# mhvk/baseband-tasks

Measured on AMD Instinct MI355X. Metric: Msamples/s through Dedisperse(DM=100)+Channelize(1k ch), 2-pol c64, higher is better.
Workload: dtype c64; 1 GPU; configs[1]+metric pipeline: Dedisperse DM=100, 16 MHz BW at 1000 MHz, 2^20-sample overlap-save blocks (836100 valid) -> Channelize(1024), 2-pol complex64, HBM-resident input; n_fft=1048576, n_chan=1024, streams_per_gpu=2, outputs=left sharded on the ranks (value); with_gather includes the all-gather

## Files before the change

### baseband-tasks_amd/csrc/bbt_hip.hip

```cpp
#include <hip/hip_runtime.h>
#include <dlfcn.h>
#include <rccl/rccl.h>

#include <algorithm>
#include <chrono>
#include <cmath>
#include <cstdarg>
#include <cstdio>
#include <cstdlib>
#include <cstring>
#include <initializer_list>
#include <map>
#include <mutex>
#include <string>
#include <tuple>
#include <vector>

#include "../../include/bbt_hip.h"
#include "bbt_kernels.hpp"
#include "gen_kernels.hpp"
#include "big_kernels.hpp"
#include "gen2_host.hpp"
#include "gen_host.hpp"
#include "osm_geo.hpp"
// ... 644 lines not shown
    int n2p = 0;
    long long in_plane = 0, out_plane = 0;
    float2* seam = nullptr;
    float2* seam_buf[2] = {nullptr, nullptr};
    size_t seam_bytes[2] = {0, 0};
    OsmKnobs knobs;
    std::vector<OsmLaunch> chunk_launches;

    bool timing = false;
    bool timing_isolated = false;
    std::vector<hipEvent_t> ev;
    std::vector<hipEvent_t> ev_free;
    int timing_stride = 4;
    int64_t pass_launches[3] = {0, 0, 0};
    int64_t pass_blocks[3] = {0, 0, 0};
    std::vector<int> ev_nblk;
    double acc_ms[3] = {0, 0, 0};
    int64_t launches = 0;
};

static int osm_flush_timing(bbt_osm_plan* p) {
    for (size_t i = 0; i + 3 < p->ev.size(); i += 4) {
        HIP_TRY(hipEventSynchronize(p->ev[i + 3]));
        for (int k = 0; k < 3; ++k) {
            float ms = 0.f;
            HIP_TRY(hipEventElapsedTime(&ms, p->ev[i + k], p->ev[i + k + 1]));
            p->acc_ms[k] += ms;
            p->pass_launches[k] += 1;
            p->pass_blocks[k] += p->ev_nblk[i / 4];
        }
        p->launches += 1;
    }
    for (auto e : p->ev) p->ev_free.push_back(e);
    p->ev.clear();
    p->ev_nblk.clear();
    return 0;
}

static_assert(fft_lds_elems(256) == FftGeo<256>::LDS_ELEMS && fft_lds_elems(512) == FftGeo<512>::LDS_ELEMS &&
                  fft_lds_elems(1024) == FftGeo<1024>::LDS_ELEMS && fft_lds_elems(2048) == FftGeo<2048>::LDS_ELEMS &&
                  fft_lds_elems(4096) == FftGeo<4096>::LDS_ELEMS && big_lds_elems(8192) == BigGeo<8192>::LDS_ELEMS &&
                  big_lds_elems(16384) == BigGeo<16384>::LDS_ELEMS && sizeof(v2) == 8 && sizeof(f4) == 16,
              "osm_launch.hpp: the exchange areas are not the templates'");

static int osm_dispatch(bbt_osm_plan* p, const OsmLaunch& l, const float2* in, float2* out, float2* work,
                        const OsmChunk& ch, const OsmChunk& chw, const SpecOut& so, hipStream_t st) {
    const dim3 grid(l.gx, l.gy), block(l.threads);
    const int S = l.single ? 1 : p->S;
#define BBT_GO(KERNEL_, ...)                                                      \
    {                                                                             \
        if (l.raise_lds && ensure_dyn_lds((const void*)KERNEL_, l.lds)) return 1; \
        hipLaunchKernelGGL(KERNEL_, grid, block, l.lds, st, __VA_ARGS__);         \
        return 0;                                                                 \
    }
    switch (l.family) {
        case OSM_COL16:
#define BBT_COL16(FIRST_, SPEC_, SINGLE_, PP_)                                      \
    if (l.first == FIRST_ && l.spec == SPEC_ && l.single == SINGLE_ && l.pp == PP_) \
        BBT_GO((k_osm_col16<FIRST_, SPEC_, SINGLE_, PP_>), in, out, work, ch, S, p->n2, so)
            BBT_COL16(true, false, true, 1) BBT_COL16(true, false, false, 8) BBT_COL16(true, false, false, 1)
            BBT_COL16(false, true, true, 1) BBT_COL16(false, false, true, 1) BBT_COL16(false, true, false, 8)
            BBT_COL16(false, false, false, 8) BBT_COL16(false, true, false, 1) BBT_COL16(false, false, false, 1)
#undef BBT_COL16
            break;
        case OSM_COL256: {
            SpecOut so_tw = so;
            if (l.tw) {
                so_tw.twa = p->twa;
                so_tw.twg = p->twg;
            }
#define BBT_COL256(FIRST_, SPEC_, F_, DET_, PP_, SINGLE_, N1_)                                                           \
    if (l.first == FIRST_ && l.spec == SPEC_ && l.F == F_ && l.det == DET_ && l.pp == PP_ && l.single == SINGLE_ &&      \
        l.n == N1_)                                                                                                      \
        BBT_GO((k_osm_col256<FIRST_, SPEC_, F_, DET_, PP_, SINGLE_, N1_>), in, out, work, ch, S, l.row_len, p->tab1.tw0, \
               so_tw, N1_ == 256 ? nullptr : p->tab1.tw1)
#define BBT_COL256_PASS(FIRST_, SPEC_)                                                                     \
    BBT_COL256(FIRST_, SPEC_, 8, false, 1, true, 512) BBT_COL256(FIRST_, SPEC_, 8, false, 1, false, 512)   \
    BBT_COL256(FIRST_, SPEC_, 8, false, 1, true, 1024) BBT_COL256(FIRST_, SPEC_, 8, false, 1, false, 1024) \
    BBT_COL256(FIRST_, SPEC_, 16, false, 1, true, 256) BBT_COL256(FIRST_, SPEC_, 16, false, 1, false, 256) \
    BBT_COL256(FIRST_, SPEC_, (FIRST_ ? 64 : 32), false, 8, false, 256)
            BBT_COL256_PASS(true, false) BBT_COL256_PASS(false, true) BBT_COL256_PASS(false, false)
            BBT_COL256(false, true, 16, true, 1, false, 256)
            BBT_COL256(true, false, 64, false, 4, false, 256)
            BBT_COL256(false, true, 16, false, 4, false, 256) BBT_COL256(false, false, 16, false, 4, false, 256)
#undef BBT_COL256_PASS
#undef BBT_COL256
            break;
        }
        case OSM_ROWPASS:
#define BBT_RP(N2_, NCH_)                                                                                           \
    if (l.n == N2_ && l.nch == NCH_)                                                                                \
        BBT_GO((k_osm_rowpass<N2_, NCH_>), work, p->n1, p->resp, p->resp_index, p->npair, p->tab2.tw0, p->tab2.tw1, \
               p->wroot, chw, p->outer, l.y0, p->tw4row, p->tw4base, p->tw_col ? (NCH_ ? 1 : 3) : 0, p->tw4o, p->tw4u)
            BBT_RP(256, 0) BBT_RP(512, 0) BBT_RP(1024, 0) BBT_RP(2048, 0) BBT_RP(4096, 0)
            BBT_RP(256, 2) BBT_RP(256, 4) BBT_RP(256, 8) BBT_RP(512, 2) BBT_RP(512, 4) BBT_RP(512, 8)
            BBT_RP(1024, 2) BBT_RP(1024, 4) BBT_RP(1024, 8) BBT_RP(2048, 2) BBT_RP(2048, 4) BBT_RP(2048, 8)
            BBT_RP(4096, 2) BBT_RP(4096, 4) BBT_RP(4096, 8)
            BBT_RP(256, 16) BBT_RP(256, 32) BBT_RP(256, 64) BBT_RP(256, 128)
            BBT_RP(512, 16) BBT_RP(512, 32) BBT_RP(512, 64) BBT_RP(512, 128)
            BBT_RP(1024, 16) BBT_RP(1024, 32) BBT_RP(1024, 64) BBT_RP(1024, 128)
            BBT_RP(2048, 16) BBT_RP(2048, 32) BBT_RP(2048, 64) BBT_RP(2048, 128)
            BBT_RP(4096, 16) BBT_RP(4096, 32) BBT_RP(4096, 64) BBT_RP(4096, 128)
            BBT_RP(256, 256)
            BBT_RP(512, 256) BBT_RP(512, 512)
            BBT_RP(1024, 256) BBT_RP(1024, 512) BBT_RP(1024, 1024)
            BBT_RP(2048, 256) BBT_RP(2048, 512) BBT_RP(2048, 1024) BBT_RP(2048, 2048)
            BBT_RP(4096, 256) BBT_RP(4096, 512) BBT_RP(4096, 1024) BBT_RP(4096, 2048) BBT_RP(4096, 4096)
#undef BBT_RP
            return fail("osm: no row pass for row length %d with %d channels", l.n, l.nch);
        case OSM_MID16:
            if (l.first) BBT_GO((k_osm_mid16<true>), work, p->n2, (int)p->n, p->wroot, l.mid_mode, l.y0)
            BBT_GO((k_osm_mid16<false>), work, p->n2, (int)p->n, p->wroot, l.mid_mode, l.y0)
        case OSM_SMALL:
#define BBT_SM(N_, PP_, SINGLE_)                         \
    if (l.n == N_ && l.pp == PP_ && l.single == SINGLE_) \
        BBT_GO((k_osm_small<N_, PP_, SINGLE_>), in, out, ch, S, p->resp, p->resp_index, p->tab2.tw0, p->tab2.tw1)
#define BBT_SM_N(N_) BBT_SM(N_, 1, true) BBT_SM(N_, 1, false) BBT_SM(N_, 2, false) BBT_SM(N_, 4, false)
            BBT_SM_N(256) BBT_SM_N(512) BBT_SM_N(1024) BBT_SM_N(2048) BBT_SM_N(4096)
            BBT_SM(256, 8, false) BBT_SM(512, 8, false) BBT_SM(1024, 8, false) BBT_SM(2048, 8, false)
#undef BBT_SM_N
#undef BBT_SM
            break;
        case OSM_SMALL_BIG:
#define BBT_SB(N_, SINGLE_)               \
    if (l.n == N_ && l.single == SINGLE_) \
        BBT_GO((k_osm_small_big<N_, SINGLE_>), in, out, ch, S, p->resp, p->resp_index, p->big_tw)
            BBT_SB(8192, true) BBT_SB(8192, false) BBT_SB(16384, true) BBT_SB(16384, false)
#undef BBT_SB
            break;
        case OSM_GEN_SMALL:
            BBT_GO(k_gen_osm_small, in, out, ch, p->S, p->resp, p->resp_index, p->g2, p->wn2, p->g2r, p->wn2r)
        case OSM_GEN_COL:
            if (l.first) BBT_GO((k_gen_col<true>), in, out, work, ch, p->S, p->n2, p->gen_ct, p->g1, p->wn1)
            BBT_GO((k_gen_col<false>), in, out, work, ch, p->S, p->n2, p->gen_ct, p->g1, p->wn1)
        case OSM_GEN_ROW:
            BBT_GO(k_gen_row, work, p->n1, p->resp, p->resp_index, p->npair, p->g2, p->wn2, p->g2r, p->wn2r, p->tlo,
                   p->thi, p->tws)
        case OSM_G2_SMALL:
            return g2_launch(p->k2_small, grid, block, st, (const float2*)in, out, ch, p->S, (const cf*)p->resp,
                             (const int*)p->resp_index, (const cf*)p->qw2, (const cf*)p->qw2r);
        case OSM_G2_FIRST:
        case OSM_G2_LAST:
            return g2_launch(l.family == OSM_G2_FIRST ? p->k2_first : p->k2_last, grid, block, st, (const float2*)in, out,
                             work, ch, p->S, p->n2, p->n2p, (const cf*)p->qw1);
        case OSM_G2_ROW:
            return g2_launch(p->k2_row, grid, block, st, work, p->n1, p->n2p, (const cf*)p->resp,
                             (const int*)p->resp_index, p->npair, (const cf*)p->qw2, (const cf*)p->qw2r,
                             (const cf*)p->tlo, (const cf*)p->thi, (const cf*)p->tws);
    }
#undef BBT_GO
    return fail("osm: no %s kernel for this plan (%d, %d pairs per workgroup, %d columns)", osm_family_name(l.family),
                l.n, l.pp, l.F);
}

static int osm_run_chunk(bbt_osm_plan* p, const float2* in, float2* out, const OsmChunk& ch_given,
                         const SpecOut& so, float2* work, hipStream_t st, bool sample = true) {
    OsmChunk ch = ch_given;
    ch.in_plane = p->in_plane;
    ch.out_plane = p->out_plane;
    hipEvent_t e[4] = {nullptr, nullptr, nullptr, nullptr};
    const bool timed = p->timing && sample;
    if (timed) {
        for (int i = 0; i < 4; ++i) {
            if (!p->ev_free.empty()) {
                e[i] = p->ev_free.back();
                p->ev_free.pop_back();
// ... 3614 lines not shown
```

### baseband-tasks_amd/csrc/bbt_kernels.hpp

```cpp
#pragma once
#include <hip/hip_runtime.h>
#include "fft_core.hpp"
#include "osm_chunk.hpp"

#ifndef BBT_SHORT_TW_POW
#define BBT_SHORT_TW_POW 1
#endif
#ifndef BBT_SMALL_TW_POW
#define BBT_SMALL_TW_POW 2
#endif
#ifndef BBT_ROWS_TW_POW
#define BBT_ROWS_TW_POW 0
#endif
#ifndef BBT_COL_TW_POW
#define BBT_COL_TW_POW 0
#endif
#ifndef BBT_ROWPASS_TW_POW
#define BBT_ROWPASS_TW_POW 2
#endif
#ifndef BBT_PFB_TW_POW
#define BBT_PFB_TW_POW 2
#endif

namespace bbt {
// ... 337 lines not shown
        v[4 * m + 3] = twmul<SIGN>(v[4 * m + 3], cmul(t2, g));
    }
}

__device__ __forceinline__ int small_channel_slot(int pos, const SpecOut& so) {
    if (so.tiny_lg) {
        const int c = pos & ((1 << so.tiny_lg) - 1);
        return pos - c + (int)(__brev((unsigned)c) >> (32 - so.tiny_lg));
    }
    if (!so.small_l) return pos;
    const int L = so.small_l, N2 = so.small_row, T = N2 >> 4;
    const int row = pos / N2, p = pos - row * N2;
    const int a = p / T, t = p - a * T;
    const int q = t / L, c = t - q * L;
    const int r = L == 1 ? 0 : (int)(__brev((unsigned)c) >> (32 - (31 - __clz(L))));
    return row * N2 + q * so.n_chan + a + 16 * r;
}

__device__ __forceinline__ float4 detect_pair(c2 z, int mode) {
    float4 p;
    p.x = z.re.x * z.re.x + z.im.x * z.im.x;
    p.y = z.re.y * z.re.y + z.im.y * z.im.y;
    p.z = mode ? z.re.x * z.re.y + z.im.x * z.im.y : 0.f;
    p.w = mode ? z.im.x * z.re.y - z.re.x * z.im.y : 0.f;
    return p;
}
__device__ __forceinline__ long long detect_index(long long bin, int ch, int sp, int lg_chan,
                                                  int npair, int mode) {
    return (((bin << lg_chan) + ch) * npair + sp) * (mode ? 4 : 2);
}
#define BBT_DET_MAX_BINS 64

struct SpecCursor {
    float2* dst;
    long long dstride;
    float2* seam0;
    float2* seam1;
    int rel, drel;
    int wrap_at;
    int n_fft, nch, vc;
    long long s0, ds, n_out;
    bool nt;
};
__device__ __forceinline__ SpecCursor spec_cursor(float2* __restrict__ out, const SpecOut& so,
                                                  const OsmBlock& blk, int row0, int row_step,
                                                  int N2, int slot, int S, int sp, int npair) {
    SpecCursor c;
    const int lg = so.lg_chan;
    c.nch = 1 << lg;
    const int ch = slot & (c.nch - 1);
    c.n_fft = so.n_fft;
    c.vc = blk.valid_count;
    c.rel = row0 * N2 + (slot - ch) + blk.shift - blk.valid_start;
    c.drel = row_step * N2;
    c.wrap_at = so.n_fft - c.nch - blk.valid_start + 1;
    c.s0 = ((blk.out_off + c.rel) >> lg) - so.s_base;
    c.ds = (long long)c.drel >> lg;
    c.n_out = so.n_out;
    c.nt = S == 2;
    c.dst = out + (((c.s0 << lg) + ch) * S + 2 * sp);
    c.dstride = ((c.ds << lg)) * S;
    c.seam0 = so.seam + (((((long long)blk.index * 2 + 0) * npair + sp) << lg) + ch) * 2;
    c.seam1 = so.seam + (((((long long)blk.index * 2 + 1) * npair + sp) << lg) + ch) * 2;
    return c;
}
__device__ __forceinline__ void emit_spectrum(c2 val, const SpecCursor& c, int j) {
    int rel = c.rel + j * c.drel;
    if (rel >= c.wrap_at) {
        if (rel < c.vc) st_ext(c.seam1, val);
        rel -= c.n_fft;
        if (rel < 0 && rel + c.nch > 0) st_ext(c.seam0, val);
        return;
    }
    if (rel >= 0 && rel + c.nch <= c.vc) {
        const long long s = c.s0 + j * c.ds;
        if (s >= 0 && s < c.n_out) st_ext(c.dst + j * c.dstride, val, c.nt);
    } else if (rel < 0 && rel + c.nch > 0) {
        st_ext(c.seam0, val);
    } else if (rel < c.vc && rel + c.nch > c.vc) {
        st_ext(c.seam1, val);
    }
}

__device__ __forceinline__ void emit_spectrum_single(float2 val, const SpecCursor& c, int j) {
    const c2 padded = c2{v2{val.x, 0.f}, v2{val.y, 0.f}};
    int rel = c.rel + j * c.drel;
    if (rel >= c.wrap_at) {
        if (rel < c.vc) st_ext(c.seam1, padded);
        rel -= c.n_fft;
        if (rel < 0 && rel + c.nch > 0) st_ext(c.seam0, padded);
        return;
    }
    if (rel >= 0 && rel + c.nch <= c.vc) {
        const long long s = c.s0 + j * c.ds;
        if (s >= 0 && s < c.n_out) c.dst[j * c.dstride] = val;
    } else if (rel < 0 && rel + c.nch > 0) {
        st_ext(c.seam0, padded);
    } else if (rel < c.vc && rel + c.nch > c.vc) {
        st_ext(c.seam1, padded);
    }
}

struct SinglePair {
    OsmBlock a, b;
    bool has_b;
};
__device__ __forceinline__ SinglePair single_pair(const OsmChunk& ch, int q) {
    SinglePair sp;
    sp.a = osm_block(ch, 2 * q);
    sp.has_b = 2 * q + 1 < (ch.reg_count ? ch.reg_count : ch.nblk);
    sp.b = osm_block(ch, sp.has_b ? 2 * q + 1 : 2 * q);
    return sp;
}
__device__ __forceinline__ c2 ld_single(const float2* __restrict__ in, const SinglePair& sp, long long e) {
    const float2 a = in[sp.a.in_off + e];
    const float2 b = sp.has_b ? in[sp.b.in_off + e] : make_float2(0.f, 0.f);
    return c2{v2{a.x, b.x}, v2{a.y, b.y}};
}
__device__ __forceinline__ c2 ld_single_shifted(const float2* __restrict__ in, const SinglePair& sp, long long e,
                                                long long n) {
    long long ea = e + sp.a.shift, eb = e + sp.b.shift;
    ea -= ea >= n ? n : 0;
    eb -= eb >= n ? n : 0;
    const float2 a = in[sp.a.in_off + ea];
    const float2 b = sp.has_b ? in[sp.b.in_off + eb] : make_float2(0.f, 0.f);
    return c2{v2{a.x, b.x}, v2{a.y, b.y}};
}
__device__ __forceinline__ void st_single(float2* __restrict__ out, const SinglePair& sp, long long e, c2 v) {
    const long long ra = e - sp.a.valid_start, rb = e - sp.b.valid_start;
    if (ra >= 0 && ra < sp.a.valid_count) out[sp.a.out_off + ra] = make_float2(v.re.x, v.im.x);
    if (sp.has_b && rb >= 0 && rb < sp.b.valid_count) out[sp.b.out_off + rb] = make_float2(v.re.y, v.im.y);
}

template <int STRIDE>
__device__ __forceinline__ void apply_resp(c2 (&v)[16], const cf* __restrict__ h0,
                                           const cf* __restrict__ h1, bool same) {
    if (same) {
#pragma unroll
        for (int j = 0; j < 16; ++j) v[j] = twmul<-1>(v[j], h0[STRIDE * j]);
    } else {
#pragma unroll
        for (int j = 0; j < 16; ++j) {
            const cf x = h0[STRIDE * j], y = h1[STRIDE * j];
            v[j] = cmul2(v[j], c2{v2{x.x, y.x}, v2{x.y, y.y}});
        }
    }
}

template <int N, int PP, bool SINGLE = false>
__global__ __launch_bounds__(PP* N / 16) void k_osm_small(const float2* __restrict__ in,
                                                          float2* __restrict__ out, OsmChunk ch, int S,
                                                          const cf* __restrict__ resp,
                                                          const int* __restrict__ resp_index,
                                                          const cf* __restrict__ tw0,
                                                          const cf* __restrict__ tw1) {
    typedef FftGeo<N> G;
    constexpr int T = G::T;
    constexpr int CM = PP > 1 ? PP : 0;
    extern __shared__ v2 osm_small_lds[];
    v2* lds = osm_small_lds;
    const unsigned vb = xcd_remap(blockIdx.x, gridDim.x);
    c2 v[16];
    if constexpr (SINGLE) {
        const int tau = threadIdx.x;
        const SinglePair pr = single_pair(ch, vb);
#pragma unroll
// ... 55 lines not shown
                                                   float2* __restrict__ work, OsmChunk ch, int S,
                                                   int N2, SpecOut so) {
    const int npair = SINGLE ? 1 : S >> 1;
    const unsigned vb = xcd_remap(blockIdx.x, gridDim.x);
    constexpr int COLS = 256 / PP;
    const int npg = npair / PP;
    const int n2 = (vb / npg) * COLS + threadIdx.x / PP;
    const int b = blockIdx.y, sp = (vb % npg) * PP + threadIdx.x % PP;
    float2* w = work + ((long long)(b * npair + sp) * 16) * N2 * 2 + (long long)n2 * 2;
    c2 v[16];
    if constexpr (SINGLE) {
        const SinglePair pr = single_pair(ch, b);
        if (FIRST) {
#pragma unroll
            for (int j = 0; j < 16; ++j)
                v[j] = ld_single_shifted(in, pr, (long long)j * N2 + n2, 16ll * N2);
            radix16<-1>(v);
#pragma unroll
            for (int j = 0; j < 16; ++j) st_int(w + (long long)j * N2 * 2, v[j]);
        } else {
#pragma unroll
            for (int j = 0; j < 16; ++j) v[j] = ld_int(w + (long long)j * N2 * 2);
            radix16<+1>(v);
            if constexpr (SPEC) {
                const SpecCursor ca = spec_cursor(out, so, pr.a, 0, 1, N2, n2, 1, 0, 1);
                const SpecCursor cb = spec_cursor(out, so, pr.b, 0, 1, N2, n2, 1, 0, 1);
#pragma unroll
                for (int j = 0; j < 16; ++j) {
                    emit_spectrum_single(make_float2(v[j].re.x, v[j].im.x), ca, j);
                    if (pr.has_b) emit_spectrum_single(make_float2(v[j].re.y, v[j].im.y), cb, j);
                }
            } else {
#pragma unroll
                for (int j = 0; j < 16; ++j) st_single(out, pr, (long long)j * N2 + n2, v[j]);
            }
        }
        return;
    }
    const OsmBlock blk = osm_block(ch, b);
    if (FIRST) {
        const float2* src = in + ((blk.in_off + n2 + blk.shift) * S + 2 * sp);
        const long long wrap = (n2 + blk.shift >= N2) ? (long long)16 * N2 * S : 0;
        if (S == 2) {
#pragma unroll
            for (int j = 0; j < 16; ++j) v[j] = ld_ext_nt(src + (long long)j * N2 * S - (j == 15 ? wrap : 0));
        } else {
#pragma unroll
            for (int j = 0; j < 16; ++j) v[j] = ld_ext(src + (long long)j * N2 * S - (j == 15 ? wrap : 0));
        }
        radix16<-1>(v);
#pragma unroll
        for (int j = 0; j < 16; ++j) st_int(w + (long long)j * N2 * 2, v[j]);
    } else {
#pragma unroll
        for (int j = 0; j < 16; ++j) v[j] = ld_int(w + (long long)j * N2 * 2);
        radix16<+1>(v);
        SpecCursor cur;
        if (SPEC) cur = spec_cursor(out, so, blk, 0, 1, N2, small_channel_slot(n2, so), S, sp, npair);
#pragma unroll
        for (int j = 0; j < 16; ++j) {
            if (SPEC) {
                emit_spectrum(v[j], cur, j);
            } else {
                const int r = j * N2 + n2 - blk.valid_start;
                if (r >= 0 && r < blk.valid_count)
                    st_ext(out + ((blk.out_off + r) * S + 2 * sp), v[j], S == 2);
            }
        }
    }
}

template <bool FIRST, bool SPEC, int FCOL, bool DET = false, int PP = 1, bool SINGLE = false, int N1 = 256>
__global__ __launch_bounds__(FCOL * (N1 / 16)) void k_osm_col256(const float2* __restrict__ in,
                                                          float2* __restrict__ out,
                                                          float2* __restrict__ work, OsmChunk ch,
                                                          int S, int N2, const cf* __restrict__ tw0,
                                                          SpecOut so, const cf* __restrict__ tw1 = nullptr) {
    typedef FftGeo<N1> G;
    constexpr int T1 = N1 / 16;
    static_assert(!DET || N1 == 256, "fused detection: 256-point columns");
    extern __shared__ v2 col256_lds[];
    v2* lds = col256_lds;
    static_assert(!DET || PP == 1, "fused detection needs the lanes of a row in one stream pair");
    const int f = threadIdx.x % FCOL, tau = threadIdx.x / FCOL;
    const int npair = SINGLE ? 1 : S >> 1;
    const unsigned vb = xcd_remap(blockIdx.x, gridDim.x);
    constexpr int CPT = FCOL / PP;
    const int npg = npair / PP;
    const int n2 = (vb / npg) * CPT + f / PP;
    const int b = blockIdx.y, sp = (vb % npg) * PP + f % PP;
    float2* w = work + (((long long)(b * npair + sp) * N1 + tau) * N2 + n2) * 2;
    c2 v[16];
    if constexpr (SINGLE) {
        static_assert(!DET && PP == 1, "one-stream plans: no fused detection");
        const SinglePair pr = single_pair(ch, b);
        if (FIRST) {
#pragma unroll
            for (int j = 0; j < 16; ++j)
                v[j] = ld_single_shifted(in, pr, (long long)(tau + T1 * j) * N2 + n2, (long long)N1 * N2);
            wg_fft<N1, -1, FCOL, 0, BBT_COL_TW_POW>(v, lds, tau, f, tw0, tw1);
            if (so.twa) col_twiddles<-1>(v, so.twa, so.twg, tau, n2, N2);
#pragma unroll
            for (int j = 0; j < 16; ++j) st_int(w + (long long)T1 * j * N2 * 2, v[j]);
        } else {
#pragma unroll
            for (int j = 0; j < 16; ++j) v[j] = ld_int(w + (long long)T1 * j * N2 * 2);
            if (so.twa) col_twiddles<+1>(v, so.twa, so.twg, tau, n2, N2);
            wg_fft<N1, +1, FCOL, 0, BBT_COL_TW_POW>(v, lds, tau, f, tw0, tw1);
            if constexpr (SPEC) {
                const SpecCursor ca = spec_cursor(out, so, pr.a, tau, T1, N2, n2, 1, 0, 1);
                const SpecCursor cb = spec_cursor(out, so, pr.b, tau, T1, N2, n2, 1, 0, 1);
#pragma unroll
                for (int j = 0; j < 16; ++j) {
                    emit_spectrum_single(make_float2(v[j].re.x, v[j].im.x), ca, j);
                    if (pr.has_b) emit_spectrum_single(make_float2(v[j].re.y, v[j].im.y), cb, j);
                }
            } else {
#pragma unroll
                for (int j = 0; j < 16; ++j) st_single(out, pr, (long long)(tau + T1 * j) * N2 + n2, v[j]);
            }
        }
        return;
    }
    const OsmBlock blk = osm_block(ch, b);
    if (FIRST) {
        const int Si = ch.in_plane ? 2 : S;
        const float2* src = in + (ch.in_plane ? (long long)sp * ch.in_plane * 2 : 2 * sp) +
                            (blk.in_off + (long long)tau * N2 + n2 + blk.shift) * Si;
        const long long wrap = (tau == T1 - 1 && n2 + blk.shift >= N2) ? (long long)N1 * N2 * Si : 0;
        if (Si == 2) {
#pragma unroll
            for (int j = 0; j < 16; ++j)
                v[j] = ld_ext_nt(src + (long long)T1 * j * N2 * 2 - (j == 15 ? wrap : 0));
        } else if (S == 2) {
#pragma unroll
            for (int j = 0; j < 16; ++j)
                v[j] = ld_ext_nt(src + (long long)T1 * j * N2 * S - (j == 15 ? wrap : 0));
        } else {
#pragma unroll
            for (int j = 0; j < 16; ++j)
                v[j] = ld_ext(src + (long long)T1 * j * N2 * S - (j == 15 ? wrap : 0));
        }
        wg_fft<N1, -1, FCOL, 0, BBT_COL_TW_POW>(v, lds, tau, f, tw0, tw1);
        if (so.twa) col_twiddles<-1>(v, so.twa, so.twg, tau, n2, N2);
#pragma unroll
        for (int j = 0; j < 16; ++j) st_int(w + (long long)T1 * j * N2 * 2, v[j]);
    } else {
#pragma unroll
        for (int j = 0; j < 16; ++j) v[j] = ld_int(w + (long long)T1 * j * N2 * 2);
        if (so.twa) col_twiddles<+1>(v, so.twa, so.twg, tau, n2, N2);
        wg_fft<N1, +1, FCOL, 0, BBT_COL_TW_POW>(v, lds, tau, f, tw0, tw1);
        SpecCursor cur;
        if (SPEC) cur = spec_cursor(out, so, blk, tau, T1, N2, small_channel_slot(n2, so), S, sp, npair);
        if constexpr (SPEC && DET) {
            constexpr int NT = FCOL * 16;
            float2* pw = reinterpret_cast<float2*>(lds);
            static_assert(256 * FCOL * 8 <= G::LDS_ELEMS * FCOL * (int)sizeof(v2),
                          "power tile does not fit the exchange buffer");
            const int step = so.det_step, mode = so.det_mode;
            const int spr = N2 >> so.lg_chan;
            const int lg_spr = __ffs(spr) - 1;
            const long long s_wg = cur.s0 - (long long)tau * spr;
            long long b_wg = s_wg / step;
            if (b_wg * step > s_wg) --b_wg;
            const long long n_bins = cur.n_out / step;
            const int ch0 = (n2 - f) & (cur.nch - 1);
            const int nb = (int)((s_wg + 255ll * spr) / step - b_wg) + 1;
            float4 p[16];
            unsigned whole = 0;
#pragma unroll
            for (int j = 0; j < 16; ++j) {
                int rel = cur.rel + j * cur.drel;
                bool full = false;
                if (rel >= cur.wrap_at) {
                    if (rel < cur.vc) st_ext(cur.seam1, v[j]);
                    rel -= cur.n_fft;
                    if (rel < 0 && rel + cur.nch > 0) st_ext(cur.seam0, v[j]);
                } else if (rel >= 0 && rel + cur.nch <= cur.vc) {
                    full = true;
                } else if (rel < 0 && rel + cur.nch > 0) {
                    st_ext(cur.seam0, v[j]);
                } else if (rel < cur.vc && rel + cur.nch > cur.vc) {
                    st_ext(cur.seam1, v[j]);
                }
                const long long sj = cur.s0 + j * cur.ds;
                const bool mine = full && sj >= 0 && sj < cur.n_out;
                whole |= (unsigned)mine << j;
                p[j] = mine ? detect_pair(v[j], mode) : make_float4(0.f, 0.f, 0.f, 0.f);
            }
            if (step == 1) {
#pragma unroll
                for (int j = 0; j < 16; ++j) {
                    if (!((whole >> j) & 1)) continue;
                    float* dst = so.det + detect_index(cur.s0 + j * cur.ds, ch0 + f, sp, so.lg_chan, npair, mode);
                    if (mode)
                        *reinterpret_cast<float4*>(dst) = make_float4(p[j].x * so.det_scale, p[j].y * so.det_scale,
                                                                      p[j].z * so.det_scale, p[j].w * so.det_scale);
                    else
                        *reinterpret_cast<float2*>(dst) = make_float2(p[j].x * so.det_scale, p[j].y * so.det_scale);
                }
                return;
            }
            const int npass = mode ? 2 : 1;
            for (int pass = 0; pass < npass; ++pass) {
                __syncthreads();
#pragma unroll
                for (int j = 0; j < 16; ++j)
                    pw[(tau + 16 * j) * FCOL + f] = pass ? make_float2(p[j].z, p[j].w)
                                                         : make_float2(p[j].x, p[j].y);
                __syncthreads();
                const float* pf = reinterpret_cast<const float*>(pw);
                for (int i = threadIdx.x; i < nb * FCOL * 2; i += NT) {
                    const int bl = i / (FCOL * 2), fc = i - bl * (FCOL * 2);
                    const long long bin = b_wg + bl;
                    if (bin < 0 || bin >= n_bins) continue;
                    const int d0 = (int)(bin * step - s_wg);
                    int lo = d0 > 0 ? (d0 + spr - 1) >> lg_spr : 0;
                    int hi = (d0 + step + spr - 1) >> lg_spr;
                    if (hi > 256) hi = 256;
                    float sum = 0.f;
                    for (int n1 = lo; n1 < hi; ++n1) sum += pf[n1 * (FCOL * 2) + fc];
                    if (sum != 0.f)
                        unsafeAtomicAdd(so.det + detect_index(bin, ch0 + (fc >> 1), sp, so.lg_chan, npair, mode)
                                            + 2 * pass + (fc & 1),
                                        sum * so.det_scale);
                }
            }
            return;
        }
#pragma unroll
        for (int j = 0; j < 16; ++j) {
            if (SPEC) {
                emit_spectrum(v[j], cur, j);
            } else {
// ... 974 lines not shown
```

### baseband-tasks_amd/csrc/osm_geo.hpp

```cpp
#pragma once
#include <algorithm>
#include <cstdarg>
#include <cstdint>
#include <cstdio>
#include <cstdlib>
#include <cstring>
#include <string>
#include <vector>

#include "gen_host.hpp"
#include "osm_limits.hpp"

namespace bbt {

static inline bool is_pow2(int64_t n) { return n > 0 && (n & (n - 1)) == 0; }
static inline bool fft_len_ok(int64_t n) { return is_pow2(n) && n >= 256 && n <= 4096; }
static inline bool is_7smooth(int64_t n) {
    if (n < 1) return false;
    for (int r : {2, 3, 5, 7})
        while (n % r == 0) n /= r;
    return n == 1;
}

static inline int rtc_mode() {
    const char* e = getenv("BBT_RTC");
    if (!e || !*e) return 1;
    if (!strcmp(e, "0")) return 0;
    if (!strcmp(e, "require")) return 2;
    return 1;
}
struct OsmKnobs {
    int rtc = 1;
    bool no_big = false;
    int64_t gen_n1 = 0;
    int gen_ct = 0;
    int lanes = 2;
    bool has_chunk = false;
    int chunk = 0;
    int timing_stride = 4;
    int small_cap = -1;
    int mid_mib = 128;
};
static inline OsmKnobs osm_knobs_from_env() {
    OsmKnobs k;
    k.rtc = rtc_mode();
    k.no_big = getenv("BBT_OSM_NO_BIG") != nullptr;
    if (const char* env = getenv("BBT_GEN_N1")) k.gen_n1 = atoll(env);
    if (const char* env = getenv("BBT_GEN_CT")) k.gen_ct = std::max(1, atoi(env));
    if (const char* env = getenv("BBT_OSM_LANES")) k.lanes = atoi(env);
    if (const char* env = getenv("BBT_OSM_CHUNK")) {
        k.has_chunk = true;
        k.chunk = atoi(env);
    }
    if (const char* env = getenv("BBT_OSM_TIMING_STRIDE")) k.timing_stride = std::max(1, atoi(env));
    if (const char* env = getenv("BBT_SMALL_CAP")) k.small_cap = std::max(0, atoi(env));
    if (const char* env = getenv("BBT_OSM_MID_MIB")) k.mid_mib = atoi(env);
    return k;
}

static inline bool split_7smooth(int64_t n, const OsmKnobs& k, int* n1, int* n2, bool* measured = nullptr) {
    const int64_t d = k.gen_n1;
    if (d > 1 && n % d == 0 && n / d <= BBT_GEN_MAX_LEN && d <= BBT_GEN_MAX_LEN) {
        if (measured) *measured = false;
        *n1 = (int)d;
        *n2 = (int)(n / d);
        return true;
    }
    return gen_split(n, k.rtc != 0, n1, n2, measured);
}

struct OsmGeo {
    int64_t n = 0;
    int S = 0, npair = 0;
    bool fast = false;
    bool generic = false;
    bool single = false;
    int outer = 1;
    int n1 = 1, n2 = 0;
    bool measured = false;
    GenGeo g1 = {}, g2 = {};
    int gen_ct = 1;
    int row_ct = 1;
    bool compiled = false;
    G2Plan q1, q2, q2r;
    int n2p = 0;
    size_t per_block = 0;
    int lanes = 1, chunk = 1, cap = 1;
    size_t work_bytes = 0;
};

static inline bool osm_refuse(std::string* error, const char* fmt, ...) {
    char buf[512];
    va_list ap;
    va_start(ap, fmt);
    vsnprintf(buf, sizeof buf, fmt, ap);
    va_end(ap);
    *error = buf;
    return false;
}

static inline bool osm_levels(int64_t n_fft, int n_stream, const OsmKnobs& k, OsmGeo* geo, std::string* error) {
    OsmGeo g;
    error->clear();
    g.fast = is_pow2(n_fft) && n_fft >= 256 && n_fft <= (1 << 24);
    int gn1 = 1, gn2 = 0;
    if (!(g.fast || (is_7smooth(n_fft) && n_fft >= 2 &&
                     (n_fft <= BBT_GEN_MAX_LEN || split_7smooth(n_fft, k, &gn1, &gn2, &g.measured)))))
        return osm_refuse(error,
                          "bbt_osm_plan_create: n_fft=%lld must be a power of two in [256, 2^24] or a product of "
                          "2, 3, 5, 7 that is <= 8192 or splits into two such factors",
                          (long long)n_fft);
    g.single = n_stream == 1 && g.fast;
    if (!(g.single || (n_stream >= 2 && n_stream % 2 == 0 && n_stream <= 65535 * 2)))
        return osm_refuse(error,
                          "bbt_osm_plan_create: n_stream=%d must be even and >= 2 (or 1 with a power-of-two block "
                          "length)", n_stream);
    g.n = n_fft;
    g.S = n_stream;
    g.npair = g.single ? 1 : n_stream / 2;
    if (!g.fast) {
        g.generic = true;
        g.n1 = n_fft <= BBT_GEN_MAX_LEN ? 1 : gn1;
    } else if (n_fft <= 4096 ||
               ((n_fft == 8192 || n_fft == 16384) && (g.single || (n_stream / 2) % 8 != 0) && !k.no_big)) {
        g.n1 = 1;
    } else if (n_fft <= (1 << 16)) {
        g.n1 = 16;
    } else if (n_fft <= (1 << 20)) {
        g.n1 = 256;
    } else if (n_fft == (1 << 21)) {
        g.n1 = 512;
    } else if (n_fft == (1 << 22) && (g.single || (n_stream / 2) % 8 != 0)) {
        g.n1 = 1024;
    } else {
        g.outer = 256;
        g.n1 = 16;
        if (n_stream / 2 > 255)
            return osm_refuse(error, "bbt_osm_plan_create: blocks longer than 2^20 support at most 510 streams");
    }
// ... 110 lines not shown
```

### baseband-tasks_amd/csrc/osm_launch.hpp

```cpp
#pragma once
#include "osm_geo.hpp"

namespace bbt {

constexpr int fft_lds_elems(int n) {
    const int r2 = n / 256, t = n / 16;
    const int pad0 = r2 < 16 ? t + r2 : t + 16;
    const int pb1 = 16 + (r2 == 2 ? 8 : r2 == 4 ? 4 : r2 == 8 ? 2 : r2 == 16 ? 1 : 0);
    int pc1 = r2 * pb1;
    while (pc1 % 32 != 16) ++pc1;
    return 16 * pad0 > 16 * pc1 ? 16 * pad0 : 16 * pc1;
}
constexpr int big_lds_elems(int n) {
    const int m = n / 256, l = m / 16;
    const int p1 = 16 * (m + 2), p3 = 256 * l + 2;
    return (p1 > p3 ? p1 : p3) * 16;
}
constexpr size_t OSM_LDS_MAX = 160 * 1024;

enum OsmFamily {
    OSM_COL16, OSM_COL256, OSM_ROWPASS, OSM_MID16, OSM_SMALL, OSM_SMALL_BIG,
    OSM_GEN_SMALL, OSM_GEN_COL, OSM_GEN_ROW,
    OSM_G2_SMALL, OSM_G2_FIRST, OSM_G2_ROW, OSM_G2_LAST
};
static inline const char* osm_family_name(int f) {
    static const char* const names[] = {"k_osm_col16", "k_osm_col256", "k_osm_rowpass", "k_osm_mid16", "k_osm_small",
                                        "k_osm_small_big", "k_gen_osm_small", "k_gen_col", "k_gen_row", "k_small",
                                        "k_first", "k_row", "k_last"};
    return names[f];
}
struct OsmLaunch {
    int family = 0;
    bool first = false;
    bool spec = false;
    int F = 0;
    int pp = 1;
    int n = 0;
    bool single = false;
    bool det = false;
    int nch = 0;
    unsigned gx = 1, gy = 1;
    int threads = 0;
    size_t lds = 0;
    bool raise_lds = false;
    int row_len = 0;
    int y0 = 0, ny = 0;
    int mid_mode = 0;
    bool tw = false;
    int mark = 0;
};

struct OsmLaunchPlan {
    int64_t n = 0;
    bool generic = false, rtc = false, single = false;
    int outer = 1, n1 = 1, n2 = 0, n2p = 0, npair = 0, S = 0, gen_ct = 1;
    int q1_threads = 0, q1_ct = 1, q2_threads = 0, q2_ct = 1;
    bool tw_col = false;
};
struct OsmChunkFacts {
    int nblk = 0, reg_count = 0;
    int n_chan = 0;
    bool det = false;
    bool in_plane = false;
    bool timing = false;
};

namespace osm_launch_detail {
struct Maker {
    const OsmLaunchPlan& p;
    const OsmChunkFacts& c;
    std::vector<OsmLaunch>* out;
    int nblkw() const { return p.single ? (c.nblk + 1) / 2 : c.nblk; }

    OsmLaunch& add(int family, unsigned gx, unsigned gy, int threads, size_t lds, bool raise_lds = false) {
        OsmLaunch l;
        l.family = family;
        l.gx = gx;
        l.gy = gy;
        l.threads = threads;
        l.lds = lds;
        l.raise_lds = raise_lds;
        l.single = p.single;
        out->push_back(l);
        return out->back();
    }

    const char* col256(bool first, bool spec, int row_len) {
        const size_t lds1 = fft_lds_elems(256) * 8;
        const int nblk = c.nblk, npair = p.npair;
        OsmLaunch* l;
        if (p.n1 == 512 || p.n1 == 1024) {
            if (c.det) return "osm: fused detection needs 256-point columns";
            const int F = 8;
            l = &add(OSM_COL256, p.single ? row_len / F : row_len / F * npair, p.single ? (nblk + 1) / 2 : nblk,
                     F * (p.n1 / 16), (size_t)fft_lds_elems(p.n1) * 8 * F, true);
            l->F = F;
        } else if (p.single) {
            if (c.det) return "osm: one-stream plans have no fused detection";
            l = &add(OSM_COL256, row_len / 16, (nblk + 1) / 2, 256, 16 * lds1);
            l->F = 16;
        } else if (spec && !first && c.det) {
            l = &add(OSM_COL256, row_len / 16 * npair, nblk, 256, 16 * lds1);
            l->F = 16;
            l->det = true;
        } else if (first && c.in_plane) {
            l = &add(OSM_COL256, row_len / 16 * npair, nblk, 256, 16 * lds1);
            l->F = 16;
        } else if (npair % 8 == 0) {
            const int F = first ? 64 : 32;
            l = &add(OSM_COL256, row_len / (F / 8) * (npair / 8), nblk, F * 16, F * lds1, true);
            l->F = F;
            l->pp = 8;
        } else if (first && npair % 4 == 0 && npair >= 8) {
            l = &add(OSM_COL256, row_len / 16 * (npair / 4), nblk, 1024, 64 * lds1, true);
            l->F = 64;
            l->pp = 4;
        } else if (!first && npair % 4 == 0) {
            l = &add(OSM_COL256, row_len / 4 * (npair / 4), nblk, 256, 16 * lds1);
            l->F = 16;
            l->pp = 4;
        } else {
            const size_t col_pad = (first && npair == 1) ? 9216 : 0;
            l = &add(OSM_COL256, row_len / 16 * npair, nblk, 256, 16 * lds1 + col_pad, col_pad != 0);
            l->F = 16;
        }
        l->first = first;
        l->spec = spec;
        l->n = (p.n1 == 512 || p.n1 == 1024) ? p.n1 : 256;
        l->row_len = row_len;
        l->tw = p.tw_col && p.outer == 1 && (first || !spec);
        return nullptr;
    }

    void col16(bool first) {
        OsmLaunch& l = add(OSM_COL16, p.n2 / 256 * p.npair, nblkw(), 256, 0);
        l.first = first;
        l.spec = !first && c.n_chan != 0;
        l.pp = (!p.single && p.npair % 8 == 0) ? 8 : 1;
    }

    void rowpass(int y0, int ny) {
        const bool flat = p.outer == 1 && nblkw() * p.npair > 1 && (long long)p.n1 * nblkw() * p.npair < (1ll << 31);
        OsmLaunch& l = flat ? add(OSM_ROWPASS, p.n1 * nblkw() * p.npair, 1, p.n2 / 16, 0)
                            : add(OSM_ROWPASS, p.n1, ny, p.n2 / 16, 0);
        l.n = p.n2;
        l.nch = c.n_chan;
        l.y0 = y0;
        l.ny = ny;
    }

    void mid16(bool first, int y0, int ny) {
        OsmLaunch& l = add(OSM_MID16, p.n2 / 256, ny, 256, 0);
        l.first = first;
        l.mid_mode = (!first && c.n_chan) ? 1 : 0;
        l.y0 = y0;
        l.ny = ny;
    }

    static int small_cap(int n) { return n <= 512 ? 8 : (n <= 2048 ? 4 : 2); }

    const char* small(const OsmKnobs& k) {
        const int n = p.n2;
        const int nblk = c.reg_count ? c.reg_count : c.nblk;
        if (n == 8192 || n == 16384) {
            OsmLaunch& l = add(OSM_SMALL_BIG, p.single ? (nblk + 1) / 2 : nblk * p.npair, 1, n / 16,
                               (size_t)big_lds_elems(n) * 8, true);
            l.n = n;
            l.mark = 3;
            return nullptr;
        }
        if (!fft_len_ok(n)) {
            static thread_local char text[64];
            snprintf(text, sizeof text, "osm: unsupported n_fft %lld", (long long)p.n);
            return text;
        }
        const size_t lds1 = (size_t)fft_lds_elems(n) * 8;
        int pp = 1;
        if (!p.single) {
            const int cap = k.small_cap >= 0 ? k.small_cap : small_cap(n);
            for (int q = 8; q > 1 && pp == 1; q /= 2)
                if (q * n / 16 <= 1024 && lds1 * q <= OSM_LDS_MAX && q <= cap && p.npair % q == 0) pp = q;
        }
        OsmLaunch& l = add(OSM_SMALL, p.single ? (nblk + 1) / 2 : nblk * (p.npair / pp), 1, pp * n / 16, lds1 * pp, pp > 1);
        l.n = n;
        l.pp = pp;
        l.mark = 3;
        return nullptr;
    }

    const char* generic() {
        if (c.n_chan) return "osm: the fused channelizer needs a power-of-two block length";
        const int nblk = c.nblk, npair = p.npair;
        if (p.n1 == 1) {
            if (p.rtc) add(OSM_G2_SMALL, nblk * npair, 1, p.q2_threads, 0).mark = 3;
            else add(OSM_GEN_SMALL, nblk * npair, 1, gen_threads(p.n2), (size_t)p.n2 * 16, true).mark = 3;
            return nullptr;
        }
        const int ct = p.gen_ct, tiles = (p.n2 + ct - 1) / ct;
        if (p.rtc) {
            add(OSM_G2_FIRST, (unsigned)tiles * npair * nblk, 1, p.q1_threads, 0).mark = 1;
            add(OSM_G2_ROW, (p.n1 + p.q2_ct - 1) / p.q2_ct, nblk * npair, p.q2_threads, 0).mark = 2;
            add(OSM_G2_LAST, (unsigned)tiles * npair * nblk, 1, p.q1_threads, 0);
            return nullptr;
        }
        if (!(ct >= 1 && (ct & (ct - 1)) == 0 && (long long)p.n1 * ct <= BBT_GEN_MAX_LEN)) {
            static thread_local char text[192];
            snprintf(text, sizeof text,
                     "osm: a column tile of %d x %d elements is more than the general kernels' %d (or not a power of two of columns)",
                     p.n1, ct, BBT_GEN_MAX_LEN);
            return text;
        }
        const size_t lds_c = (size_t)p.n1 * ct * 16, lds_r = (size_t)p.n2 * 16;
        OsmLaunch& a = add(OSM_GEN_COL, tiles * npair, nblk, gen_threads(p.n1 * ct), lds_c, true);
        a.first = true;
        a.mark = 1;
        add(OSM_GEN_ROW, p.n1, nblk * npair, gen_threads(p.n2), lds_r, true).mark = 2;
        add(OSM_GEN_COL, tiles * npair, nblk, gen_threads(p.n1 * ct), lds_c, true);
        return nullptr;
    }

    const char* three_levels(const OsmKnobs& k) {
        const int m_len = 16 * p.n2;
        const int rows_all = nblkw() * p.npair * 256;
        const long long mid_bytes = (long long)k.mid_mib << 20;
        const long long row_bytes = 16ll * p.n2 * 16;
        int step = mid_bytes > 0 ? (int)std::max<long long>(1, mid_bytes / row_bytes) : rows_all;
        if (c.timing) step = rows_all;
        if (const char* no = col256(true, false, m_len)) return no;
        for (int y0 = 0; y0 < rows_all; y0 += step) {
            const int ny = std::min(step, rows_all - y0);
            mid16(true, y0, ny);
            out->back().mark = 1;
            rowpass(y0, ny);
            out->back().mark = 2;
            mid16(false, y0, ny);
        }
        return col256(false, c.n_chan != 0, m_len);
    }

    const char* two_levels() {
        if (p.n1 == 16) col16(true);
        else if (const char* no = col256(true, false, p.n2)) return no;
        out->back().mark = 1;
        rowpass(0, nblkw() * p.npair);
        out->back().mark = 2;
        if (p.n1 == 16) col16(false);
        else return col256(false, c.n_chan != 0, p.n2);
        return nullptr;
    }
};
}

static inline const char* osm_chunk_launches(const OsmLaunchPlan& p, const OsmChunkFacts& c, const OsmKnobs& k,
                                             std::vector<OsmLaunch>* out) {
    out->clear();
    osm_launch_detail::Maker m{p, c, out};
    if (p.generic) return m.generic();
    if (p.n1 == 1) return m.small(k);
    if (p.outer > 1) return m.three_levels(k);
    return m.two_levels();
}

}
```

Before: 51760 Msamples/s.

## Widen last spectral column pass to 64 lanes with wave-uniform output cursor

For the final (spectral) 256-point column pass with 8 stream pairs per tile, the tile width goes from 32 to 64 columns, with an env knob to override it. A new specialization makes the row index wave-uniform via readfirstlane and splits the spectrum output cursor into a wave-uniform part and a small per-lane part. It also skips the column twiddles on this path. The intent is to cut per-lane address arithmetic and register pressure in the store epilogue and to amortize work over larger tiles, at the cost of more LDS per block (64 tiles) and possibly lower occupancy.

Result: no change. 51790 Msamples/s, median of 2 (+0.0%).

```diff
diff --git a/baseband-tasks_amd/csrc/bbt_hip.hip b/baseband-tasks_amd/csrc/bbt_hip.hip
--- a/baseband-tasks_amd/csrc/bbt_hip.hip
+++ b/baseband-tasks_amd/csrc/bbt_hip.hip
@@ -750,6 +750,7 @@
             BBT_COL256_PASS(true, false) BBT_COL256_PASS(false, true) BBT_COL256_PASS(false, false)
             BBT_COL256(false, true, 16, true, 1, false, 256)
             BBT_COL256(true, false, 64, false, 4, false, 256)
+            BBT_COL256(false, true, 64, false, 8, false, 256)
             BBT_COL256(false, true, 16, false, 4, false, 256) BBT_COL256(false, false, 16, false, 4, false, 256)
 #undef BBT_COL256_PASS
 #undef BBT_COL256
diff --git a/baseband-tasks_amd/csrc/bbt_kernels.hpp b/baseband-tasks_amd/csrc/bbt_kernels.hpp
--- a/baseband-tasks_amd/csrc/bbt_kernels.hpp
+++ b/baseband-tasks_amd/csrc/bbt_kernels.hpp
@@ -443,6 +443,76 @@
     }
 }
 
+#ifndef BBT_STREAM_NT8
+#define BBT_STREAM_NT8 0
+#endif
+
+struct SpecCursorWave {
+    float2* dst;
+    long long dstride;
+    float2* seam0;
+    float2* seam1;
+    int r0, drel, wrap_at, n_fft, nch, vc;
+    long long a0;
+    long long span;
+    bool nt;
+};
+struct SpecCursorLane {
+    int g;
+    unsigned off;
+    unsigned seam;
+};
+__device__ __forceinline__ float2* spec_at(float2* base, unsigned bytes) {
+    return reinterpret_cast<float2*>(reinterpret_cast<char*>(base) + bytes);
+}
+__device__ __forceinline__ SpecCursorWave spec_cursor_wave(float2* __restrict__ out, const SpecOut& so,
+                                                           const OsmBlock& blk, int row0, int row_step,
+                                                           int N2, int S, int npair) {
+    SpecCursorWave c;
+    const int lg = so.lg_chan;
+    c.nch = 1 << lg;
+    c.n_fft = so.n_fft;
+    c.vc = blk.valid_count;
+    c.r0 = row0 * N2 + blk.shift - blk.valid_start;
+    c.drel = row_step * N2;
+    c.wrap_at = so.n_fft - c.nch - blk.valid_start + 1;
+    c.a0 = blk.out_off + c.r0 - (so.s_base << lg);
+    c.span = so.n_out << lg;
+    c.nt = S == 2 || BBT_STREAM_NT8;
+    c.dst = out + c.a0 * S;
+    c.dstride = (long long)c.drel * S;
+    c.seam0 = so.seam + ((((long long)blk.index * 2 + 0) * npair) << lg) * 2;
+    c.seam1 = so.seam + ((((long long)blk.index * 2 + 1) * npair) << lg) * 2;
+    return c;
+}
+__device__ __forceinline__ SpecCursorLane spec_cursor_lane(const SpecOut& so, int slot, int S, int sp) {
+    SpecCursorLane c;
+    const int ch = slot & ((1 << so.lg_chan) - 1);
+    c.g = slot - ch;
+    c.off = (unsigned)(slot * S + 2 * sp) * 8u;
+    c.seam = (unsigned)(((sp << so.lg_chan) + ch) * 2) * 8u;
+    return c;
+}
+__device__ __forceinline__ void emit_spectrum(c2 val, const SpecCursorWave& c, const SpecCursorLane& l, int j) {
+    int rel = c.r0 + j * c.drel + l.g;
+    if (rel >= c.wrap_at) {
+        if (rel < c.vc) st_ext(spec_at(c.seam1, l.seam), val);
+        rel -= c.n_fft;
+        if (rel < 0 && rel + c.nch > 0) st_ext(spec_at(c.seam0, l.seam), val);
+        return;
+    }
+    if (rel >= 0 && rel + c.nch <= c.vc) {
+        const long long a = c.a0 + (long long)j * c.drel;
+        const long long lo = -a, hi = c.span - a, top = 1ll << 30;
+        const int lo32 = (int)(lo < 0 ? 0 : lo > top ? top : lo), hi32 = (int)(hi < 0 ? 0 : hi > top ? top : hi);
+        if (l.g >= lo32 && l.g < hi32) st_ext(spec_at(c.dst + j * c.dstride, l.off), val, c.nt);
+    } else if (rel < 0 && rel + c.nch > 0) {
+        st_ext(spec_at(c.seam0, l.seam), val);
+    } else if (rel < c.vc && rel + c.nch > c.vc) {
+        st_ext(spec_at(c.seam1, l.seam), val);
+    }
+}
+
 __device__ __forceinline__ void emit_spectrum_single(float2 val, const SpecCursor& c, int j) {
     const c2 padded = c2{v2{val.x, 0.f}, v2{val.y, 0.f}};
     int rel = c.rel + j * c.drel;
@@ -664,7 +734,10 @@
     extern __shared__ v2 col256_lds[];
     v2* lds = col256_lds;
     static_assert(!DET || PP == 1, "fused detection needs the lanes of a row in one stream pair");
-    const int f = threadIdx.x % FCOL, tau = threadIdx.x / FCOL;
+    constexpr bool WAVE_ROW = !FIRST && SPEC && !DET && !SINGLE && FCOL == 64 && PP == 8 && N1 == 256;
+    const int f = threadIdx.x % FCOL;
+    int tau = threadIdx.x / FCOL;
+    if constexpr (WAVE_ROW) tau = __builtin_amdgcn_readfirstlane(tau);
     const int npair = SINGLE ? 1 : S >> 1;
     const unsigned vb = xcd_remap(blockIdx.x, gridDim.x);
     constexpr int CPT = FCOL / PP;
@@ -714,7 +787,7 @@
 #pragma unroll
             for (int j = 0; j < 16; ++j)
                 v[j] = ld_ext_nt(src + (long long)T1 * j * N2 * 2 - (j == 15 ? wrap : 0));
-        } else if (S == 2) {
+        } else if (S == 2 || (BBT_STREAM_NT8 && PP == 8)) {
 #pragma unroll
             for (int j = 0; j < 16; ++j)
                 v[j] = ld_ext_nt(src + (long long)T1 * j * N2 * S - (j == 15 ? wrap : 0));
@@ -730,8 +803,18 @@
     } else {
 #pragma unroll
         for (int j = 0; j < 16; ++j) v[j] = ld_int(w + (long long)T1 * j * N2 * 2);
-        if (so.twa) col_twiddles<+1>(v, so.twa, so.twg, tau, n2, N2);
+        if constexpr (!WAVE_ROW)
+            if (so.twa) col_twiddles<+1>(v, so.twa, so.twg, tau, n2, N2);
         wg_fft<N1, +1, FCOL, 0, BBT_COL_TW_POW>(v, lds, tau, f, tw0, tw1);
+        if constexpr (WAVE_ROW) {
+            const SpecCursorWave cw = spec_cursor_wave(out, so, blk, tau, T1, N2, S, npair);
+            const SpecCursorLane cl = spec_cursor_lane(so, small_channel_slot(n2, so), S, sp);
+#pragma unroll
+            for (int j = 0; j < 16; ++j) asm volatile("" : "+v"(v[j].re), "+v"(v[j].im));
+#pragma unroll
+            for (int j = 0; j < 16; ++j) emit_spectrum(v[j], cw, cl, j);
+            return;
+        }
         SpecCursor cur;
         if (SPEC) cur = spec_cursor(out, so, blk, tau, T1, N2, small_channel_slot(n2, so), S, sp, npair);
         if constexpr (SPEC && DET) {
diff --git a/baseband-tasks_amd/csrc/osm_geo.hpp b/baseband-tasks_amd/csrc/osm_geo.hpp
--- a/baseband-tasks_amd/csrc/osm_geo.hpp
+++ b/baseband-tasks_amd/csrc/osm_geo.hpp
@@ -40,6 +40,7 @@
     int timing_stride = 4;
     int small_cap = -1;
     int mid_mib = 128;
+    int col_last_f = 0;
 };
 static inline OsmKnobs osm_knobs_from_env() {
     OsmKnobs k;
@@ -55,6 +56,7 @@
     if (const char* env = getenv("BBT_OSM_TIMING_STRIDE")) k.timing_stride = std::max(1, atoi(env));
     if (const char* env = getenv("BBT_SMALL_CAP")) k.small_cap = std::max(0, atoi(env));
     if (const char* env = getenv("BBT_OSM_MID_MIB")) k.mid_mib = atoi(env);
+    if (const char* env = getenv("BBT_COL_LAST_F")) k.col_last_f = atoi(env) == 32 || atoi(env) == 64 ? atoi(env) : 0;
     return k;
 }
 
diff --git a/baseband-tasks_amd/csrc/osm_launch.hpp b/baseband-tasks_amd/csrc/osm_launch.hpp
--- a/baseband-tasks_amd/csrc/osm_launch.hpp
+++ b/baseband-tasks_amd/csrc/osm_launch.hpp
@@ -17,6 +17,7 @@
     return (p1 > p3 ? p1 : p3) * 16;
 }
 constexpr size_t OSM_LDS_MAX = 160 * 1024;
+static_assert(64 * fft_lds_elems(256) * 8 <= OSM_LDS_MAX, "the 64-lane tiles of the 256-point column passes");
 
 enum OsmFamily {
     OSM_COL16, OSM_COL256, OSM_ROWPASS, OSM_MID16, OSM_SMALL, OSM_SMALL_BIG,
@@ -69,6 +70,7 @@
 struct Maker {
     const OsmLaunchPlan& p;
     const OsmChunkFacts& c;
+    const OsmKnobs& knobs;
     std::vector<OsmLaunch>* out;
     int nblkw() const { return p.single ? (c.nblk + 1) / 2 : c.nblk; }
 
@@ -107,7 +109,8 @@
             l = &add(OSM_COL256, row_len / 16 * npair, nblk, 256, 16 * lds1);
             l->F = 16;
         } else if (npair % 8 == 0) {
-            const int F = first ? 64 : 32;
+            int F = first || spec ? 64 : 32;
+            if (!first && spec && knobs.col_last_f) F = knobs.col_last_f;
             l = &add(OSM_COL256, row_len / (F / 8) * (npair / 8), nblk, F * 16, F * lds1, true);
             l->F = F;
             l->pp = 8;
@@ -254,7 +257,7 @@
 static inline const char* osm_chunk_launches(const OsmLaunchPlan& p, const OsmChunkFacts& c, const OsmKnobs& k,
                                              std::vector<OsmLaunch>* out) {
     out->clear();
-    osm_launch_detail::Maker m{p, c, out};
+    osm_launch_detail::Maker m{p, c, k, out};
     if (p.generic) return m.generic();
     if (p.n1 == 1) return m.small(k);
     if (p.outer > 1) return m.three_levels(k);
```
